# gmum/3d-point-clouds-autocomplete

Hardware: AMD Instinct MI355X
Metric: train-step point-clouds/sec at B=64, N=2048 (Chamfer+EMD) (higher is better)
Workload: dtype f32 storage / accumulation / results; matrix products formed from f16 x2 (bf16 x3) pieces of the fp32 operands — NOT IEEE-fp32 products: the all-fp32-kernel step is `value_strict_fp32`

## Files before the change

3d-point-clouds-autocomplete_amd/csrc/hp_skinny.h:

```cpp
#pragma once
#include <hip/hip_runtime.h>

#define HP_SK_MAX_OPS 16

enum { HP_SK_F = 1, HP_SK_X = 2, HP_SK_W = 3, HP_SK_FIN = 4 };

typedef struct HpSkSrc {
    const float* p;
    long slab;
    const float* bias;
    const float* mask;
    float* mat;
    int S, ld, ldm, ldmat, relu;
} HpSkSrc;

typedef struct HpSkOp {
    int type, phase;
    HpSkSrc a;
    const float* w;
    float* out;
    long out_slab;
    const float* out_bias;
    float* rsum;
    int w_ld, out_ld, out_relu;
    int M, N, K, CL;
    int ntasks;
} HpSkOp;

typedef struct HpSkProgram {
    int nops;
    HpSkOp op[HP_SK_MAX_OPS];
} HpSkProgram;

#ifdef __cplusplus
int hp_skinny_run(HpSkProgram* prog, hipStream_t stream);
int hp_skinny_check(HpSkProgram* prog);
bool hp_skinny_enabled();
#endif
```

3d-point-clouds-autocomplete_amd/csrc/model.hip:

```cpp
#include "hp_common.h"
#include "hp_gemm.h"
#include "hp_conv_split.h"
#include "hp_model.h"
#include "hp_skinny.h"
#include "hp_enc_bwd.h"
#include <algorithm>
#include <cstdlib>

extern "C" int hp_gemm_f32(const HpGemmDesc* d, hipStream_t stream);
extern "C" int hp_gemm_tile_rows(const HpGemmDesc* d);
extern "C" int hp_colsum_f32(int batch, int M, int N, const float* X, long sXz, int ldx, const float* mask, long sMaskz,
                             int ldmask, float* out, long sOz, float* ws, hipStream_t stream);

namespace {

constexpr int kEnc[6] = {3, 64, 128, 256, 512, 512};
constexpr int kTrunk[5] = {64, 128, 512, 1024, 2048};
constexpr long kSplitWs = 4L << 20;

#define TRY(x)            \
    do {                  \
        int _rc = (x);    \
        if (_rc) return _rc; \
    } while (0)
// ... 913 lines not shown
                                  const HpEncoderGrads* gr, float* ws, const float* fwd_ws, int dedup, hipStream_t stream) {
    const HpEncoderBwdIO io{x, w, eps, argidx, g, f, lv, grad_out, grad_mu, grad_explv, gr, ws, fwd_ws, is_vae, grad_out_ld};
    return encoder_backward_impl(B, Np, out_size, 1, &io, dedup, stream);
}
HP_API int hp_encoder_backward(int B, int Np, const float* x, const HpEncoderWeights* w, int out_size, int is_vae,
                               const float* eps, const int* argidx, const float* g, const float* f, const float* lv,
                               const float* grad_out, const float* grad_mu, const float* grad_explv,
                               const HpEncoderGrads* gr, float* ws, const float* fwd_ws, int dedup, hipStream_t stream) {
    return hp_encoder_backward_ld(B, Np, x, w, out_size, is_vae, eps, argidx, g, f, lv, grad_out, out_size, grad_mu, grad_explv, gr, ws,
                                  fwd_ws, dedup, stream);
}
HP_API int hp_encoder_backward_set_fused(int on) { return g_enc_bwd_fused.set(on); }
HP_API int hp_encoder_backward_set_chain_f16(int on) { return hp_enc_bwd_chain_f16_set(on); }
HP_API int hp_encoder_backward_pair(int B, int Np, int out_size, const HpEncoderBwdIO* io, int dedup, hipStream_t stream) {
    return encoder_backward_impl(B, Np, out_size, 2, io, dedup, stream);
}

HP_API int hp_encoder_plan(int B, int Np, int out_size, int n, const int* is_vae, const int* ld, int aligned, int dedup,
                           HpEncoderPlan* plan) {
    HP_CHECK_ARG(n >= 1 && n <= 2 && is_vae && plan && enc_fwd_shape_ok(B, Np, out_size, n));
    for (int z = 0; z < n; ++z) HP_CHECK_ARG(!ld || ld[z] == 0 || ld[z] >= out_size);
    HP_CHECK_ARG(!dedup || (long)Np * 512 < (1L << 31));
    *plan = HpEncoderPlan{};
    float* const base = reinterpret_cast<float*>(uintptr_t(1) << 40);
    const long span = 1L << 34;
    HpEncoderWeights w{};
    HpEncoderGrads gr{};
    for (int l = 0; l < 5; ++l) {
        w.conv_w[l] = w.conv_b[l] = base;
        gr.conv_w[l] = gr.conv_b[l] = base;
    }
    w.fc_w = w.fc_b = w.mu_w = w.mu_b = w.std_w = w.std_b = base;
    gr.fc_w = gr.fc_b = gr.mu_w = gr.mu_b = gr.std_w = gr.std_b = base;
    auto ld_of = [&](int z) { return (ld && ld[z] > 0) ? ld[z] : out_size; };

    const EncFwdRoute r = enc_fwd_route(B, Np, out_size, n);
    plan->conv_format = r.presplit ? HP_ENC_CONV_PFORMAT : r.split ? HP_ENC_CONV_SPLIT_F32 : HP_ENC_CONV_GEMM_F32;
    plan->pool_fused = r.fused ? 1 : 0;
    plan->tile_rows = r.tr;
    if (enc_fwd_tails_try_skinny(r, B)) {
        EncTail t[2];
        for (int z = 0; z < n; ++z) {
            const bool block = n > 1 && !is_vae[z];
            t[z] = EncTail{base, &w, is_vae[z], base, base + (block ? out_size : 0), base, base + (z + 1) * span + r.tail_off,
                           block ? ld_of(z) : out_size};
        }
        HpSkProgram pr;
        plan->fwd_tails_skinny = enc_tail_forward_program(B, out_size, n, t, pr) == 0 && hp_skinny_check(&pr) == 0;
    }

    plan->bwd_fused = (enc_bwd_shapes_fuse(B, out_size, dedup) && aligned) ? 1 : 0;
    const bool chain16 = hp_enc_bwd_chain_f16_enabled();
    plan->bwd_splits = plan->bwd_fused ? enc_bwd_splits(B, chain16) : 0;
    EncTailBwd t[2];
    bool ask = true;
    for (int z = 0; z < n; ++z) {
        const EncBwdWs L = enc_bwd_layout(base + (z + 1) * span + (aligned ? 0 : 1), B, out_size);
        const float* dmu_p = is_vae[z] ? L.dmu : base + (n > 1 ? out_size : 0);
        const int dmu_ld = is_vae[z] ? out_size : ld_of(z);
        t[z] = EncTailBwd{base, base, &w, dmu_p, dmu_ld, is_vae[z] ? L.dlv : nullptr, &gr, L.dfc, L.dg, L.split};
        ask = ask && enc_bwd_tail_try_skinny(B, dmu_p, dmu_ld);
        if (!plan->bwd_fused) {
            HpSkProgram pr;
            plan->bwd_tails_skinny[z] = enc_bwd_tail_try_skinny(B, dmu_p, dmu_ld) &&
                                        enc_tail_backward_program(B, out_size, 1, &t[z], pr) == 0 && hp_skinny_check(&pr) == 0;
        }
    }
    if (plan->bwd_fused) {
        HpSkProgram pr;
        const int ok = ask && enc_tail_backward_program(B, out_size, n, t, pr) == 0 && hp_skinny_check(&pr) == 0;
        for (int z = 0; z < n; ++z) plan->bwd_tails_skinny[z] = ok;
    }
    return 0;
}

namespace {
template <typename P>
bool heads_contiguous(P const* hw, P const* hb, const int* out, int n) {
    for (int h = 0; h + 1 < n; ++h)
        if (hw[h + 1] != hw[h] + (long)out[h] * 2048 || hb[h + 1] != hb[h] + out[h]) return false;
    return n > 0;
}

int trunk_forward_skinny(int B, int in_size, const float* latent, const HpHyperWeights* w, float* t, float* slabs,
                         hipStream_t stream) {
    if (B > 64 || in_size % 32) return -2;
    HpSkProgram pr{};
    HpSkSrc src{};
    src.p = latent; src.S = 1; src.ld = in_size;
    float* tl = t;
    float* sl = slabs;
    int kin = in_size;
    for (int l = 0; l < 5; ++l) {
        const int N = kTrunk[l];
        const int S = sk_ranges(kin, N / 32, 4);
        HpSkOp& op = pr.op[pr.nops++];
        op.type = HP_SK_F; op.phase = l;
        op.a = src;
        op.w = w->trunk_w[l]; op.w_ld = kin;
        op.M = B; op.N = N; op.K = kin; op.CL = kin / S;
        op.out_ld = N;
        HpSkSrc next{};
        next.ld = N;
        if (S == 1) {
            op.out = tl; op.out_bias = w->trunk_b[l]; op.out_relu = l < 4;
            next.p = tl; next.S = 1;
        } else {
            op.out = sl; op.out_slab = 64L * N;
            next.p = sl; next.slab = 64L * N; next.S = S; next.bias = w->trunk_b[l]; next.relu = l < 4;
            next.mat = tl; next.ldmat = N;
            sl += (long)S * 64 * N;
            if (sl - slabs > kSplitWs) return -2;
        }
        src = next;
        kin = N;
        tl += (long)B * N;
    }
    if (src.S > 1) {
        HpSkOp& op = pr.op[pr.nops++];
        op.type = HP_SK_FIN; op.phase = 5;
        op.out = src.mat; op.out_ld = src.ldmat;
        src.mat = nullptr;
        op.a = src;
        op.M = B; op.N = 2048; op.K = 1;
    }
    return hp_skinny_run(&pr, stream);
}

int trunk_backward_skinny(int B, int in_size, const float* latent, const HpHyperWeights* w, const float* const* act,
                          float* const* dt, const HpHyperGrads* gr, float* grad_latent, float* slabs, hipStream_t stream) {
    if (B > 64 || in_size % 32) return -2;
    HpSkProgram pr{};
    HpSkSrc src{};
    src.p = dt[4]; src.S = 1; src.ld = kTrunk[4];
    float* sl = slabs;
    int phase = 0;
    auto dw_op = [&](int l) {
        HpSkOp& op = pr.op[pr.nops++];
        op.type = HP_SK_W; op.phase = phase;
        op.a.p = dt[l]; op.a.S = 1; op.a.ld = kTrunk[l];
        op.w = l ? act[l - 1] : latent; op.w_ld = l ? kTrunk[l - 1] : in_size;
        op.out = gr->trunk_w[l]; op.out_ld = op.w_ld; op.rsum = gr->trunk_b[l];
        op.M = B; op.N = kTrunk[l]; op.K = op.w_ld;
    };
    for (int l = 4; l >= 0; --l, ++phase) {
        const int N = kTrunk[l], K = l ? kTrunk[l - 1] : in_size;
        if (l == 0 && !grad_latent) {
            HpSkOp& op = pr.op[pr.nops++];
            op.type = HP_SK_FIN; op.phase = phase;
            op.out = src.mat; op.out_ld = src.ldmat;
            src.mat = nullptr;
            op.a = src;
            op.M = B; op.N = N; op.K = 1;
        } else {
            const int S = sk_ranges(N, K / 32, 4);
            HpSkOp& op = pr.op[pr.nops++];
            op.type = HP_SK_X; op.phase = phase;
            op.a = src;
            op.w = w->trunk_w[l]; op.w_ld = K;
            op.M = B; op.N = N; op.K = K; op.CL = N / S;
            op.out_ld = K;
            HpSkSrc next{};
            next.ld = K;
            if (l == 0) {
                if (S == 1) {
                    op.out = grad_latent;
                } else {
                    op.out = sl; op.out_slab = 64L * K;
                    next.p = sl; next.slab = 64L * K; next.S = S;
                    sl += (long)S * 64 * K;
                }
            } else {
                op.out = sl; op.out_slab = 64L * K;
                next.p = sl; next.slab = 64L * K; next.S = S;
                next.mask = act[l - 1]; next.ldm = K; next.mat = dt[l - 1]; next.ldmat = K;
                sl += (long)S * 64 * K;
            }
            if (sl - slabs > kSplitWs) return -2;
            src = next;
        }
        if (l == 4) dw_op(4);
        else if (l <= 2) dw_op(l + 1);
    }
    if (grad_latent && src.p && src.S > 1) {
        HpSkOp& op = pr.op[pr.nops++];
        op.type = HP_SK_FIN; op.phase = phase;
        op.a = src;
        op.out = grad_latent; op.out_ld = in_size;
        op.M = B; op.N = in_size; op.K = 1;
    }
    dw_op(0);
    return hp_skinny_run(&pr, stream);
}

template <typename T>
inline T* hyper_splitws(T* t, int B) { return t + ((long)B * (64 + 128 + 512 + 1024 + 2048) + 3) / 4 * 4; }
inline int heads_total(const HpHyperWeights* w) {
    int total = 0;
    for (int hd = 0; hd < w->n_heads; ++hd) total += w->head_out[hd];
    return total;
}
int heads_fwd_route(int B, const HpHyperWeights* w, const float* t) {
    if (!heads_contiguous(w->head_w, w->head_b, w->head_out, w->n_heads)) return HP_HEADS_FWD_PER_HEAD;
    const float* t5 = t + (long)B * (64 + 128 + 512 + 1024);
    return hp_heads_fwd_enabled() && hp_heads_fwd_ws_floats() <= kSplitWs &&
                   hp_heads_fwd_ok(B, heads_total(w), 2048, t5, w->head_w[0], hyper_splitws(t, B))
               ? HP_HEADS_FWD_STREAM : HP_HEADS_FWD_GEMM;
}
int heads_dw_route(const HpHyperWeights* w, const HpHyperGrads* gr, const float* t5) {
    const bool skip_dw = gr->head_w[0] == nullptr;
    bool gb_contig = true;
    for (int h = 0; h + 1 < w->n_heads; ++h) gb_contig = gb_contig && gr->head_b[h + 1] == gr->head_b[h] + w->head_out[h];
    const bool w_contig = heads_contiguous(w->head_w, w->head_b, w->head_out, w->n_heads);
    if (skip_dw) return gb_contig && w_contig ? HP_HEADS_DW_SKIPPED : -1;
    if (!w_contig || !heads_contiguous(gr->head_w, gr->head_b, w->head_out, w->n_heads)) return HP_HEADS_DW_PER_HEAD;
    return hp_heads_dw_fast_ok(2048, t5, gr->head_w[0]) ? HP_HEADS_DW_DIRECT : HP_HEADS_DW_GEMM;
}
int heads_dw_rows_route(const float* t5_all, const float* dW_rows) {
    return hp_heads_dw_fast_ok(2048, t5_all, dW_rows) ? HP_HEADS_DW_DIRECT : HP_HEADS_DW_GEMM;
}
}

HP_API long hp_hypernet_saved_floats(int B) { return (long)B * (64 + 128 + 512 + 1024 + 2048) + kSplitWs + 64; }
HP_API long hp_hypernet_backward_workspace_floats(int B) { return (long)B * (64 + 128 + 512 + 1024 + 2048) + kSplitWs + 64; }

HP_API int hp_hypernet_set_heads_stream(int on) { return hp_heads_fwd_set(on); }

HP_API int hp_hypernet_forward(int B, int in_size, const float* latent, const HpHyperWeights* w, float* t, float* theta,
                               int theta_ld, hipStream_t stream) {
    HP_CHECK_ARG(B > 0 && in_size > 0 && latent && w && t && theta && w->n_heads > 0 && w->n_heads <= HP_MAX_HEADS);
    Op op{stream, hyper_splitws(t, B)};
    const float* in = latent;
    int kin = in_size;
    float* tl = t;
    int sk = hp_skinny_enabled() ? trunk_forward_skinny(B, in_size, latent, w, t, op.splitws, stream) : -2;
    if (sk != -2) {
        TRY(sk);
        in = t + (long)B * (64 + 128 + 512 + 1024);
    } else {
        for (int l = 0; l < 5; ++l) {
            TRY(op.lin_fwd(in, 0, kin, w->trunk_w[l], 0, w->trunk_b[l], 0, tl, 0, kTrunk[l], B, kTrunk[l], kin, 1, l < 4));
            in = tl;
            kin = kTrunk[l];
            tl += (long)B * kTrunk[l];
        }
    }
    const int total = heads_total(w);
    HP_CHECK_ARG(total <= theta_ld);
    switch (heads_fwd_route(B, w, t)) {
    case HP_HEADS_FWD_STREAM:
        TRY(hp_heads_fwd(B, total, in, w->head_w[0], w->head_b[0], theta, theta_ld, op.splitws, stream));
        break;
    case HP_HEADS_FWD_GEMM:
        TRY(op.lin_fwd(in, 0, 2048, w->head_w[0], 0, w->head_b[0], 0, theta, 0, theta_ld, B, total, 2048, 1, false));
        break;
    default: {
        int off = 0;
        for (int hd = 0; hd < w->n_heads; ++hd) {
            TRY(op.lin_fwd(in, 0, 2048, w->head_w[hd], 0, w->head_b[hd], 0, theta + off, 0, theta_ld, B, w->head_out[hd], 2048,
                           1, false));
            off += w->head_out[hd];
        }
    }
    }
    HP_RETURN_LAST_ERROR();
}

namespace {
int hypernet_backward_impl(int B, int in_size, const float* latent, const HpHyperWeights* w, const float* t, const float* grad_theta,
                           int theta_ld, const HpHyperGrads* gr, float* grad_latent, float* ws, hipStream_t stream, hipStream_t after);
}
HP_API int hp_hypernet_backward(int B, int in_size, const float* latent, const HpHyperWeights* w, const float* t,
                                const float* grad_theta, int theta_ld, const HpHyperGrads* gr, float* grad_latent, float* ws,
                                hipStream_t stream) {
    return hypernet_backward_impl(B, in_size, latent, w, t, grad_theta, theta_ld, gr, grad_latent, ws, stream, nullptr);
}
HP_API int hp_hypernet_backward_ordered(int B, int in_size, const float* latent, const HpHyperWeights* w, const float* t,
                                        const float* grad_theta, int theta_ld, const HpHyperGrads* gr, float* grad_latent, float* ws,
                                        hipStream_t stream, hipStream_t after) {
    return hypernet_backward_impl(B, in_size, latent, w, t, grad_theta, theta_ld, gr, grad_latent, ws, stream, after);
}
namespace {
int hypernet_backward_impl(int B, int in_size, const float* latent, const HpHyperWeights* w, const float* t, const float* grad_theta,
                           int theta_ld, const HpHyperGrads* gr, float* grad_latent, float* ws, hipStream_t stream, hipStream_t after) {
    HP_CHECK_ARG(B > 0 && in_size > 0 && latent && w && t && grad_theta && gr && ws);
    const float* act[5];
    {
        const float* tl = t;
        for (int l = 0; l < 5; ++l) {
            act[l] = tl;
            tl += (long)B * kTrunk[l];
        }
    }
    float* p = ws;
    float* dt[5];
    for (int l = 0; l < 5; ++l) {
        dt[l] = p;
        p += (long)B * kTrunk[l];
    }
    Op op{stream, p};
    int off = 0;
    const int total = heads_total(w);
    const int route = heads_dw_route(w, gr, act[4]);
    HP_CHECK_ARG(route >= 0);
    const bool fused = route != HP_HEADS_DW_PER_HEAD;
    if (fused) {
        if (route == HP_HEADS_DW_DIRECT) {
// ... 150 lines not shown
```

3d-point-clouds-autocomplete_amd/csrc/skinny.hip:

```cpp
#include "hp_common.h"
#include "hp_pieces.h"
#include "hp_skinny.h"
#include <algorithm>
#include <atomic>
#include <cstdlib>

namespace {

using namespace hp_pieces;
typedef int i32x4 __attribute__((ext_vector_type(4)));

constexpr int kThreads = 256;
constexpr int kCLMax = 128;
constexpr int kLdsFloats = 96 * (kCLMax + 4);

constexpr int kPhaseOps = 8;
struct Prog {
    int nops;
    HpSkOp op[kPhaseOps];
};

struct Buf {
    __amdgpu_buffer_rsrc_t r;
    __device__ __forceinline__ explicit Buf(const void* base)
        : r(__builtin_amdgcn_make_buffer_rsrc(const_cast<void*>(base), 0, 0x7fffffff, 0x00020000)) {}
    __device__ __forceinline__ float4 ld4(long off_floats) const {
        const i32x4 v = __builtin_amdgcn_raw_buffer_load_b128(r, (int)(off_floats * 4), 0, 0);
        return make_float4(__int_as_float(v.x), __int_as_float(v.y), __int_as_float(v.z), __int_as_float(v.w));
    }
    __device__ __forceinline__ float ld1(long off_floats) const {
        return __int_as_float(__builtin_amdgcn_raw_buffer_load_b32(r, (int)(off_floats * 4), 0, 0));
    }
};

__device__ __forceinline__ float4 f4add(float4 a, float4 b) { return make_float4(a.x + b.x, a.y + b.y, a.z + b.z, a.w + b.w); }
__device__ __forceinline__ float4 f4zero() { return make_float4(0.f, 0.f, 0.f, 0.f); }
__device__ __forceinline__ float f4get(const float4& v, int s) { return s == 0 ? v.x : (s == 1 ? v.y : (s == 2 ? v.z : v.w)); }

__device__ __forceinline__ float4 src_finish(const HpSkSrc& a, float4 v, const float4& aux) {
    if (a.bias) v = f4add(v, aux);
    if (a.relu) v = make_float4(fmaxf(v.x, 0.f), fmaxf(v.y, 0.f), fmaxf(v.z, 0.f), fmaxf(v.w, 0.f));
    if (a.mask) v = make_float4(aux.x > 0.f ? v.x : 0.f, aux.y > 0.f ? v.y : 0.f, aux.z > 0.f ? v.z : 0.f, aux.w > 0.f ? v.w : 0.f);
    return v;
}

__device__ __forceinline__ float4 src_load4(const HpSkSrc& a, int row, int c) {
    const Buf buf(a.p);
    const long off = (long)row * a.ld + c;
    float4 t[4];
#pragma unroll
    for (int s = 0; s < 4; ++s)
        if (s < a.S) t[s] = buf.ld4(off + (long)s * a.slab);
    float4 aux = f4zero();
    if (a.bias) aux = *reinterpret_cast<const float4*>(a.bias + c);
    if (a.mask) aux = *reinterpret_cast<const float4*>(a.mask + (long)row * a.ldm + c);
    float4 v = t[0];
#pragma unroll
    for (int s = 1; s < 4; ++s)
        if (s < a.S) v = f4add(v, t[s]);
    return src_finish(a, v, aux);
}

template <int NG, int SB>
struct SrcChunk {
    static constexpr int CL = NG * 16, ldl = CL + 4, QR = CL / 4;
    float4 t[NG][SB], aux[NG];
    int c0;
    __device__ __forceinline__ void load(const HpSkSrc& a, int M, int c0_) {
        c0 = c0_;
        const Buf buf(a.p);
        const float* auxp = a.bias ? a.bias : (a.mask ? a.mask : a.p);
        const int aux_ld = a.bias ? 0 : (a.mask ? a.ldm : a.ld);
#pragma unroll
        for (int e = 0; e < NG; ++e) {
            const int idx = threadIdx.x + e * kThreads, row = min(idx / QR, M - 1), q = idx % QR;
            const long off = (long)row * a.ld + c0 + 4 * q;
#pragma unroll
            for (int u = 0; u < SB; ++u) t[e][u] = buf.ld4(off + (long)(u < a.S ? u : 0) * a.slab);
            aux[e] = *reinterpret_cast<const float4*>(auxp + (long)row * aux_ld + c0 + 4 * q);
        }
    }
    __device__ __forceinline__ void store(const HpSkSrc& a, int M, float* As, bool materialise) const {
#pragma unroll
        for (int e = 0; e < NG; ++e) {
            const int idx = threadIdx.x + e * kThreads, row = idx / QR, q = idx % QR;
            float4 v = t[e][0];
#pragma unroll
            for (int u = 1; u < SB; ++u)
                if (u < a.S) v = f4add(v, t[e][u]);
            float4 f = src_finish(a, v, aux[e]);
            if (row >= M) f = f4zero();
            *reinterpret_cast<float4*>(&As[row * ldl + 4 * q]) = f;
            if (materialise && row < M) *reinterpret_cast<float4*>(a.mat + (long)row * a.ldmat + c0 + 4 * q) = f;
        }
    }
};

template <int NG>
struct WChunk {
    static constexpr int CL = NG * 16, ldl = CL + 4, QR = CL / 4, NV = NG / 2;
    static_assert(NV * kThreads == 32 * QR, "whole passes of the workgroup over the block");
    float4 v[NV];
    __device__ __forceinline__ void load(const float* __restrict__ W, int ld, int N, int n0, int c0) {
#pragma unroll
        for (int e = 0; e < NV; ++e) {
            const int idx = threadIdx.x + e * kThreads;
            v[e] = *reinterpret_cast<const float4*>(W + (long)min(n0 + idx / QR, N - 1) * ld + c0 + 4 * (idx % QR));
        }
    }
    __device__ __forceinline__ void store(float* Ws) const {
#pragma unroll
        for (int e = 0; e < NV; ++e) {
            const int idx = threadIdx.x + e * kThreads;
            *reinterpret_cast<float4*>(&Ws[(idx / QR) * ldl + 4 * (idx % QR)]) = v[e];
        }
    }
};

__device__ __forceinline__ void reduce_store(f32x16 (&acc)[2], float* red, const HpSkOp& op, float* out, int ncols, int col0,
                                             bool direct) {
    const int lane = threadIdx.x & 63, w = threadIdx.x >> 6, i = lane & 31, h = lane >> 5;
    __syncthreads();
#pragma unroll
    for (int mt = 0; mt < 2; ++mt)
#pragma unroll
        for (int e = 0; e < 16; ++e) red[((w * 2 + mt) * 16 + e) * 64 + lane] = acc[mt][e];
    __syncthreads();
    const int col = col0 + i;
    const float bv = (direct && op.out_bias && col < ncols) ? op.out_bias[col] : 0.f;
#pragma unroll
    for (int mt = 0; mt < 2; ++mt)
#pragma unroll
        for (int q = 0; q < 4; ++q) {
            const int e = 4 * w + q;
            float v = red[((0 * 2 + mt) * 16 + e) * 64 + lane];
            v += red[((1 * 2 + mt) * 16 + e) * 64 + lane];
            v += red[((2 * 2 + mt) * 16 + e) * 64 + lane];
            v += red[((3 * 2 + mt) * 16 + e) * 64 + lane];
            const int row = mt * 32 + cd_row(e, h);
            if (direct) {
                v += bv;
                if (op.out_relu) v = fmaxf(v, 0.f);
            }
            if (row < op.M && col < ncols) out[(long)row * op.out_ld + col] = v;
        }
    __syncthreads();
}

template <int NG, int SB>
__device__ __forceinline__ void task_f(const HpSkOp& op, int t, float* lds) {
    constexpr int CL = NG * 16, ldl = CL + 4, ks = CL / 4;
    const int strips = (op.N + 31) >> 5;
    const int strip = t % strips, range = t / strips;
    const int nr = op.K / op.CL;
    const int lane = threadIdx.x & 63, w = threadIdx.x >> 6, i = lane & 31, h = lane >> 5;
    const int chunks = op.CL / CL;
    const bool mat = strip == 0 && op.a.mat != nullptr;
    float* As = lds;
    float* Ws = lds + 64 * ldl;
    f32x16 acc[2] = {};
    SrcChunk<NG, SB> sc[2];
    WChunk<NG> wc[2];
    const int c_first = range * op.CL;
    auto mfma_chunk = [&]() {
#pragma unroll
        for (int kq = 0; kq < ks / 8; ++kq) {
            const int kk = w * ks + kq * 8;
            const float4 a0 = *reinterpret_cast<const float4*>(&As[i * ldl + kk + 4 * h]);
            const float4 a1 = *reinterpret_cast<const float4*>(&As[(32 + i) * ldl + kk + 4 * h]);
            const float4 bb = *reinterpret_cast<const float4*>(&Ws[i * ldl + kk + 4 * h]);
#pragma unroll
            for (int s = 0; s < 4; ++s) {
                acc[0] = __builtin_amdgcn_mfma_f32_32x32x2f32(f4get(a0, s), f4get(bb, s), acc[0], 0, 0, 0);
                acc[1] = __builtin_amdgcn_mfma_f32_32x32x2f32(f4get(a1, s), f4get(bb, s), acc[1], 0, 0, 0);
            }
        }
    };
    wc[0].load(op.w, op.w_ld, op.N, strip * 32, c_first);
    sc[0].load(op.a, op.M, c_first);
#pragma unroll 1
    for (int ch = 0; ch < chunks; ch += 2) {
        {
            const int c1 = c_first + min(ch + 1, chunks - 1) * CL;
            wc[1].load(op.w, op.w_ld, op.N, strip * 32, c1);
            sc[1].load(op.a, op.M, c1);
        }
        if (ch) __syncthreads();
        sc[0].store(op.a, op.M, As, mat);
        wc[0].store(Ws);
        __syncthreads();
        mfma_chunk();
        if (ch + 1 >= chunks) break;
        {
            const int c2 = c_first + min(ch + 2, chunks - 1) * CL;
            wc[0].load(op.w, op.w_ld, op.N, strip * 32, c2);
            sc[0].load(op.a, op.M, c2);
        }
// ... 36 lines not shown
#pragma unroll
            for (int s = 0; s < 4; ++s) {
                acc[0] = __builtin_amdgcn_mfma_f32_32x32x2f32(f4get(a0, s), bwc[4 * g + s], acc[0], 0, 0, 0);
                acc[1] = __builtin_amdgcn_mfma_f32_32x32x2f32(f4get(a1, s), bwc[4 * g + s], acc[1], 0, 0, 0);
            }
        }
    };
    const int n_first = range * op.CL;
    load_b(n_first, bw[0]);
    sc[0].load(op.a, op.M, n_first);
#pragma unroll 1
    for (int ch = 0; ch < chunks; ch += 2) {
        {
            const int n1 = n_first + min(ch + 1, chunks - 1) * CL;
            load_b(n1, bw[1]);
            sc[1].load(op.a, op.M, n1);
        }
        if (ch) __syncthreads();
        sc[0].store(op.a, op.M, As, mat);
        __syncthreads();
        mfma_chunk(bw[0]);
        if (ch + 1 >= chunks) break;
        {
            const int n2 = n_first + min(ch + 2, chunks - 1) * CL;
            load_b(n2, bw[0]);
            sc[0].load(op.a, op.M, n2);
        }
        __syncthreads();
        sc[1].store(op.a, op.M, As, mat);
        __syncthreads();
        mfma_chunk(bw[1]);
    }
    reduce_store(acc, lds, op, op.out + (long)range * op.out_slab, op.K, unit * 32, nr == 1);
}

__device__ __forceinline__ void task_w(const HpSkOp& op, int t) {
    const int lane = threadIdx.x & 63, w = threadIdx.x >> 6, i = lane & 31, h = lane >> 5;
    const int ktiles = (op.K + 31) >> 5, ntiles = (op.N + 31) >> 5;
    const int tile = t * 4 + w;
    if (tile >= ktiles * ntiles) return;
    const int kt = tile % ktiles, nt = tile / ktiles;
    const int ncol = min(nt * 32 + i, op.N - 1), kcol = min(kt * 32 + i, op.K - 1);
    const float* ap = op.a.p + ncol;
    const float* bp = op.w + kcol;
    float av[32], bv[32];
#pragma unroll
    for (int s = 0; s < 32; ++s) {
        const int m = min(2 * s + h, op.M - 1);
        av[s] = ap[(long)m * op.a.ld];
        bv[s] = bp[(long)m * op.w_ld];
    }
#pragma unroll
    for (int s = 0; s < 32; ++s)
        if (2 * s + h >= op.M) av[s] = 0.f;
    f32x16 acc = {};
    float asum = 0.f;
#pragma unroll
    for (int s = 0; s < 32; ++s) {
        asum += av[s];
        acc = __builtin_amdgcn_mfma_f32_32x32x2f32(av[s], bv[s], acc, 0, 0, 0);
    }
    if (op.rsum && kt == 0) {
        const float other = __shfl_xor(asum, 32, 64);
        if (h == 0 && nt * 32 + i < op.N) op.rsum[nt * 32 + i] = asum + other;
    }
    const int col = kt * 32 + i;
    if (col < op.K) {
#pragma unroll
        for (int e = 0; e < 16; ++e) {
            const int row = nt * 32 + cd_row(e, h);
            if (row < op.N) op.out[(long)row * op.out_ld + col] = acc[e];
        }
    }
}

__device__ __forceinline__ void task_fin(const HpSkOp& op, int t) {
    const int q_per_row = op.N >> 2;
    const int idx = t * kThreads + threadIdx.x;
    if (idx >= op.M * q_per_row) return;
    const int r = idx / q_per_row, q = idx - r * q_per_row;
    *reinterpret_cast<float4*>(op.out + (long)r * op.out_ld + 4 * q) = src_load4(op.a, r, 4 * q);
}

template <bool LIGHT>
__global__ __launch_bounds__(kThreads) void skinny_kernel(const Prog g_arg) {
    __shared__ __attribute__((aligned(16))) float lds[LIGHT ? 4 : kLdsFloats];
    const int G = gridDim.x;
    const Prog& g = *(const Prog*)__builtin_amdgcn_kernarg_segment_ptr();
    (void)g_arg;
    int base = 0;
    for (int o = 0; o < g.nops; ++o) {
        const HpSkOp& op = g.op[o];
        int first = (int)blockIdx.x - base % G;
        if (first < 0) first += G;
        const int cl = min(op.CL, kCLMax);
        for (int t = first; t < op.ntasks; t += G) {
            if (!LIGHT && op.type == HP_SK_F) {
                if (op.a.S == 1) {
                    if (cl == 128) task_f<8, 1>(op, t, lds);
                    else if (cl == 64) task_f<4, 1>(op, t, lds);
                    else task_f<2, 1>(op, t, lds);
                } else {
                    if (cl >= 64) task_f<4, 4>(op, t, lds);
                    else task_f<2, 4>(op, t, lds);
                }
            } else if (!LIGHT && op.type == HP_SK_X) {
                if (op.a.S == 1) {
                    if (cl == 128) task_x<8, 1>(op, t, lds);
                    else if (cl == 64) task_x<4, 1>(op, t, lds);
                    else task_x<2, 1>(op, t, lds);
                } else {
                    if (cl >= 64) task_x<4, 4>(op, t, lds);
                    else task_x<2, 4>(op, t, lds);
                }
            } else if (op.type == HP_SK_W) {
                task_w(op, t);
            } else if (op.type == HP_SK_FIN) {
                task_fin(op, t);
            }
        }
        base += op.ntasks;
    }
}

inline bool aligned16(const void* q) { return (reinterpret_cast<uintptr_t>(q) & 15) == 0; }
inline bool pow2(int v) { return v > 0 && (v & (v - 1)) == 0; }

bool src_ok(const HpSkSrc& a, int cols) {
    if (!a.p || a.S < 1 || a.S > 4 || !aligned16(a.p) || a.ld % 4 || cols % 4) return false;
    if (a.S > 1 && a.slab % 4) return false;
    if (a.bias && !aligned16(a.bias)) return false;
    if (a.mask && (!aligned16(a.mask) || a.ldm % 4)) return false;
    if (a.mat && (!aligned16(a.mat) || a.ldmat % 4)) return false;
    if (a.bias && a.mask) return false;
    return true;
}

}

namespace {
hp::Switch g_skinny("HP_SKINNY", 1);
}
bool hp_skinny_enabled() { return g_skinny.get() != 0; }
HP_API int hp_skinny_set_enabled(int on) { return g_skinny.set(on); }

namespace {
std::atomic<long> g_programs_run{0};
}
HP_API long hp_skinny_programs_run(void) { return g_programs_run.load(std::memory_order_relaxed); }

int hp_skinny_check(HpSkProgram* prog) {
    if (!prog || prog->nops < 1 || prog->nops > HP_SK_MAX_OPS) return -2;
    int maxtasks = 0, phases = 1;
    for (int o = 0; o < prog->nops; ++o) {
        HpSkOp& op = prog->op[o];
        if (o && op.phase < prog->op[o - 1].phase) return -2;
        if (o && op.phase != prog->op[o - 1].phase) ++phases;
        if (op.M < 1 || op.M > 64 || op.N < 1 || op.K < 1 || !op.out || !aligned16(op.out)) return -2;
        switch (op.type) {
            case HP_SK_F:
                if (op.K % 32 || !pow2(op.CL) || op.CL < 32 || op.K % op.CL || !src_ok(op.a, op.K) || !op.w || !aligned16(op.w) ||
                    op.w_ld % 4)
                    return -2;
                op.ntasks = ((op.N + 31) / 32) * (op.K / op.CL);
                break;
            case HP_SK_X:
                if (op.N % 32 || !pow2(op.CL) || op.CL < 32 || op.N % op.CL || !src_ok(op.a, op.N) || !op.w) return -2;
                op.ntasks = ((op.K + 31) / 32) * (op.N / op.CL);
                break;
            case HP_SK_W:
                if (!op.a.p || op.a.S != 1 || op.a.bias || op.a.mask || op.a.relu || !op.w) return -2;
                op.ntasks = (((op.N + 31) / 32) * ((op.K + 31) / 32) + 3) / 4;
                break;
            case HP_SK_FIN:
                if (op.N % 4 || op.out_ld % 4 || !src_ok(op.a, op.N)) return -2;
                op.ntasks = (op.M * (op.N / 4) + kThreads - 1) / kThreads;
                break;
            default: return -2;
        }
        maxtasks = std::max(maxtasks, op.ntasks);
    }
    (void)phases;
    (void)maxtasks;
    return 0;
}

int hp_skinny_run(HpSkProgram* prog, hipStream_t stream) {
    if (hp_skinny_check(prog)) return -2;
    g_programs_run.fetch_add(1, std::memory_order_relaxed);
    for (int b = 0; b < prog->nops;) {
        Prog g;
        g.nops = 0;
        int e = b, tasks = 0;
        bool light = true;
        for (; e < prog->nops && prog->op[e].phase == prog->op[b].phase && g.nops < kPhaseOps; ++e) {
            g.op[g.nops++] = prog->op[e];
            tasks += prog->op[e].ntasks;
            light = light && (prog->op[e].type == HP_SK_W || prog->op[e].type == HP_SK_FIN);
        }
        const dim3 grid(std::max(1, std::min(tasks, 512)));
        if (light) hipLaunchKernelGGL(skinny_kernel<true>, grid, dim3(kThreads), 0, stream, g);
        else hipLaunchKernelGGL(skinny_kernel<false>, grid, dim3(kThreads), 0, stream, g);
        b = e;
    }
    HP_RETURN_LAST_ERROR();
}
```

include/hyperpocket_hip.h:

```cpp
#ifndef HYPERPOCKET_HIP_H
#define HYPERPOCKET_HIP_H

#ifdef __cplusplus
extern "C" {
#endif

typedef struct ihipStream_t* hpStream_t;


int hp_nndistance(int b, int n, const float* xyz, int m, const float* xyz2, float* result, int* result_i,
                  float* result2, int* result2_i, hpStream_t stream);

int hp_nn_set_queries_per_lane(int r);
int hp_nn_queries_per_lane(int b, int n, int m);

int hp_nndistancegrad(int b, int n, const float* xyz1, int m, const float* xyz2, const float* grad_dist1,
                      const int* idx1, const float* grad_dist2, const int* idx2, float* grad_xyz1, float* grad_xyz2,
                      hpStream_t stream);

int hp_approxmatch(int b, int n, int m, const float* xyz1, const float* xyz2, float* match, float* temp,
                   hpStream_t stream);
long hp_approxmatch_workspace_floats(int b, int n, int m);
int hp_approxmatch_ws(int b, int n, int m, const float* xyz1, const float* xyz2, float* match, float* temp, float* ws,
                      hpStream_t stream);
// ... 142 lines not shown
int hp_conv_presplit_set(int on);
long hp_gemm_pp_workspace_floats(long M, int N, int K);
int hp_gemm_pp_prepare(long M, int N, int K, int xcb, const float* X, const float* W, float* ws, hpStream_t stream);
int hp_gemm_pp_run(long M, int N, int K, int xcb, const float* bias, int relu, int mode, int group_rows, float* ws, hpStream_t stream);
int hp_gemm_pp_unpack(long M, int N, int K, const float* ws, float* C, hpStream_t stream);
int hp_gemm_pp_partials(long M, int N, int K, const float* ws, float* cmax, int* cidx, hpStream_t stream);
int hp_gemm_pp_plan(long M, int N, int mode, int n, int out[6]);
long hp_encoder_backward_workspace_floats(int B, int out_size);
int hp_encoder_backward(int B, int Np, const float* x, const HpEncoderWeights* w, int out_size, int is_vae,
                        const float* eps, const int* argidx, const float* g, const float* f, const float* lv,
                        const float* grad_out, const float* grad_mu, const float* grad_explv, const HpEncoderGrads* grads,
                        float* ws, const float* fwd_ws, int dedup, hpStream_t stream);
int hp_encoder_backward_ld(int B, int Np, const float* x, const HpEncoderWeights* w, int out_size, int is_vae,
                           const float* eps, const int* argidx, const float* g, const float* f, const float* lv,
                           const float* grad_out, int grad_out_ld, const float* grad_mu, const float* grad_explv,
                           const HpEncoderGrads* grads, float* ws, const float* fwd_ws, int dedup, hpStream_t stream);
typedef struct HpEncoderBwdIO {
    const float* x;
    const HpEncoderWeights* w;
    const float* eps;
    const int* argidx;
    const float *g, *f, *lv;
    const float *grad_out, *grad_mu, *grad_explv;
    const HpEncoderGrads* gr;
    float* ws;
    const float* fwd_ws;
    int is_vae;
    int grad_out_ld;
} HpEncoderBwdIO;
int hp_encoder_backward_pair(int B, int Np, int out_size, const HpEncoderBwdIO* io , int dedup, hpStream_t stream);
enum { HP_ENC_CONV_PFORMAT = 0, HP_ENC_CONV_SPLIT_F32 = 1, HP_ENC_CONV_GEMM_F32 = 2 };
typedef struct HpEncoderPlan {
    int conv_format;
    int pool_fused;
    int tile_rows;
    int fwd_tails_skinny;
    int bwd_fused;
    int bwd_splits;
    int bwd_tails_skinny[2];
} HpEncoderPlan;
int hp_encoder_plan(int B, int Np, int out_size, int n, const int* is_vae, const int* ld, int aligned, int dedup,
                    HpEncoderPlan* plan);
int hp_encoder_backward_set_fused(int on);
int hp_encoder_backward_set_chain_f16(int on);
int hp_conv_split_set(int on);
long hp_gemm_f16x2_workspace_floats(long M, int N, int K);
int hp_gemm_f16x2_prepare(long M, int N, int K, const float* X, const float* W, float* ws, hpStream_t stream);
int hp_gemm_f16x2_run(long M, int N, int K, const float* X, const float* bias, float* C, int relu, const float* ws, hpStream_t stream);

int hp_hypernet_set_heads_stream(int on);
long hp_hypernet_saved_floats(int B);
int hp_hypernet_forward(int B, int in_size, const float* latent, const HpHyperWeights* w, float* t, float* theta,
                        int theta_ld, hpStream_t stream);
long hp_hypernet_backward_workspace_floats(int B);
int hp_hypernet_backward(int B, int in_size, const float* latent, const HpHyperWeights* w, const float* t,
                         const float* grad_theta, int theta_ld, const HpHyperGrads* grads, float* grad_latent ,
                         float* ws, hpStream_t stream);
int hp_hypernet_backward_ordered(int B, int in_size, const float* latent, const HpHyperWeights* w, const float* t,
                                 const float* grad_theta, int theta_ld, const HpHyperGrads* grads, float* grad_latent ,
                                 float* ws, hpStream_t stream, hpStream_t after);
long hp_hypernet_t5_offset(int B);
long hp_hypernet_heads_dw_workspace_floats(void);
int hp_hypernet_heads_dw_rows(int Kc, int rows, int r0, const float* dtheta_all, int theta_ld, const float* t5_all,
                              float* dW_rows, float* ws, hpStream_t stream);
enum { HP_HEADS_FWD_STREAM = 0, HP_HEADS_FWD_GEMM = 1, HP_HEADS_FWD_PER_HEAD = 2 };
enum { HP_HEADS_DW_DIRECT = 0, HP_HEADS_DW_GEMM = 1, HP_HEADS_DW_PER_HEAD = 2, HP_HEADS_DW_SKIPPED = 3 };
typedef struct HpHeadsPlan {
    int fwd_route;
    int dw_route;
    int dw_rows_route;
} HpHeadsPlan;
int hp_hypernet_heads_plan(int B, const HpHyperWeights* w, const HpHyperGrads* grads , const float* t,
                           const float* dW_rows , HpHeadsPlan* plan);

int hp_hypernet_heads_dw_adam(int Kc, int rows, int r0, const float* dtheta_all, int theta_ld, const float* t5_all,
                              float* W_rows, float* m_rows, float* v_rows, float lr, float beta1, float beta2, float eps,
                              int step, hpStream_t stream);
int hp_hypernet_heads_dw_adam_bg(int Kc, int rows, int r0, const float* dtheta_all, int theta_ld, const float* t5_all,
                                 float* W_rows, float* m_rows, float* v_rows, float lr, float beta1, float beta2, float eps,
                                 int step, int cus, hpStream_t stream);

int hp_skinny_set_enabled(int on);
long hp_skinny_programs_run(void);

long hp_target_theta_size(int n_hidden, const int* channels);
long hp_target_saved_floats(int B, int N, int n_hidden, const int* channels);
int hp_target_forward(int B, int N, int n_hidden, const int* channels, const float* theta, int theta_ld, const float* pts,
                      float* acts, float* y, hpStream_t stream);
long hp_target_backward_workspace_floats(int B, int N, int n_hidden, const int* channels);
int hp_target_backward(int B, int N, int n_hidden, const int* channels, const float* theta, int theta_ld, const float* pts,
                       const float* acts, const float* grad_y, float* grad_theta, float* ws, hpStream_t stream);

int hp_target_fused_supported(int n_hidden, const int* channels);
long hp_target_fused_workspace_floats(int B, int N);
int hp_target_fused_set_f16(int on);
int hp_target_fused_forward(int B, int N, const float* theta, int theta_ld, const float* pts, float* y, hpStream_t stream);
int hp_target_fused_backward(int B, int N, const float* theta, int theta_ld, const float* pts, const float* grad_y,
                             float* grad_theta, float* ws, hpStream_t stream);

int hp_sample_points(long total, float coef, unsigned long long seed, unsigned long long offset, float* out,
                     hpStream_t stream);
int hp_slice_clouds(int B, int N, int target, const float* pts, unsigned long long seed, int max_rounds, float* part_a,
                    float* part_b, float* plane, int* status, hpStream_t stream);
int hp_slice_clouds_planes(int B, int N, int target, const float* pts, const double* planes, int R, float* part_a,
                           float* part_b, int* plane_idx, int* status, hpStream_t stream);
long hp_make_batch_workspace_bytes(int B, int N);
int hp_make_batch(int M, int N, int target, const float* clouds, int B, const int* ids, const long long* streams,
                  const int* degrees, const float* rot, unsigned long long seed, int max_candidates, int groups,
                  float* existing, float* missing, float* gt, float* plane, int* index, int* failed, void* ws,
                  hpStream_t stream);
#define HP_VIEW_SPLIT_MAX_POINTS 8192
#define HP_VIEW_SPLIT_MIN_RESOLUTION 4
#define HP_VIEW_SPLIT_MAX_RESOLUTION 128
#define HP_VIEW_SPLIT_MAX_WINDOW 4
int hp_make_view_batch_plan(int N, int R, int* threads, int* lds);
int hp_make_view_batch(int M, int N, int target, const float* clouds, int B, const int* ids, const float* frames ,
                       const int* degrees, const float* rot, double dist, double scale, int R, int w, float* existing,
                       float* missing, float* gt, unsigned char* side , float* occlusion ,
                       hpStream_t stream);
#define HP_SCAN_MAX_POINTS (1 << 22)
int hp_scan_boxes(int S, const float* points, const long long* offsets, float* center , float* scale ,
                  hpStream_t stream);
int hp_prepare_scans(int B, const float* points, const long long* offsets, int S, const int* ids, const long long* streams,
                     unsigned long long seed, int target, int replace, const float* center, const float* scale, float* out,
                     int* index, int* failed, hpStream_t stream);
int hp_restore_scans(int K, int N, const float* completions, const float* s_scale, const float* center, const float* scale,
                     float* out, hpStream_t stream);
#define HP_FPS_MAX_POINTS 8192
int hp_farthest_points(int B, int P, const float* clouds, const int* counts, const int* start, int k, int* index,
                       float* radius2, int* failed, hpStream_t stream);
int hp_farthest_points_plan(int P, int* threads, int* points_per_lane);
#define HP_KNN_MAX_POINTS 65536
int hp_knn_points(int S, const float* points, const long long* offsets, const float* queries, const long long* query_offsets,
                  int k, int exclude_self, int* index , float* dist2 , hpStream_t stream);
int hp_knn_points_plan(int k, int* instance_k, int* threads, int* tile);
int hp_scan_outliers(int S, const float* points, const long long* offsets, int k, float ratio, unsigned char* keep ,
                     float* mean_dist , int* kept , hpStream_t stream);
#define HP_KNN_GRID_MAX_POINTS (1 << 22)
long long hp_knn_grid_workspace_bytes(int S, long long T, long long Q);
int hp_knn_grid_plan(int k, int* instance_k, int* threads, int* tile);
int hp_knn_grid(int S, const float* points, const long long* offsets, const float* queries, const long long* query_offsets,
                int k, int exclude_self, const float* cell , int* index , float* dist2 ,
                float* mean_dist , float* grid , void* ws, long long ws_bytes,
                hpStream_t stream);
int hp_outlier_keep(int S, const float* mean_dist, const long long* offsets, float ratio, unsigned char* keep ,
                    int* kept , hpStream_t stream);
int hp_scan_outliers_grid(int S, const float* points, const long long* offsets, int k, float ratio, const float* cell,
                          unsigned char* keep , float* mean_dist , int* kept , void* ws,
                          long long ws_bytes, hpStream_t stream);
#define HP_CLUSTER_MAX_POINTS 32768
int hp_scan_clusters(int S, const float* points, const long long* offsets, float radius, int max_points,
                     int* label , int* size , int* clusters , int* largest ,
                     hpStream_t stream);
int hp_scan_clusters_plan(int max_points, int* threads, int* tile, int* lds_bytes);
#define HP_PLANE_MAX_TRIALS 4096
long hp_scan_plane_workspace_bytes(int S, int trials);
int hp_scan_plane_plan(int trials, int* threads, int* rows_per_lane, int* trial_tile);
int hp_scan_plane(int S, const float* points, const long long* offsets, const long long* streams ,
                  unsigned long long seed, int trials, float threshold, int min_inliers, float min_share,
                  int* trial , int* inliers , int* found , int* sample ,
                  float* sample_plane , unsigned char* inlier , long long* moments ,
                  int* shift , void* ws, hpStream_t stream);
int hp_scan_plane_side(int S, const float* points, const long long* offsets, const float* planes , float threshold,
                       float* dist , unsigned char* keep , int* kept , hpStream_t stream);
#define HP_VOXEL_GRID_HALF (1 << 20)
long hp_scan_voxels_workspace_bytes(long long T, int slots_per_row);
// ... 112 lines not shown
```

Baseline: 28790.

## Specialize skinny kernel instances per phase body set to cut LDS and raise occupancy

Replaces the two-way light/heavy skinny kernel with six template instances. Each instance compiles only the task bodies its launch phase actually uses, and sizes its LDS allocation and launch-bounds occupancy hint to match. Phases that use only small-CL bodies can then keep two workgroups per CU with a smaller LDS footprint instead of the worst-case 96x132 buffer. It also adds a planning API for inspecting which instance each launch picks. The costs are more compiled kernel variants and the risk that the tighter launch bounds raise register pressure or cause spills for the larger bodies.

```diff
diff --git a/3d-point-clouds-autocomplete_amd/csrc/hp_skinny.h b/3d-point-clouds-autocomplete_amd/csrc/hp_skinny.h
--- a/3d-point-clouds-autocomplete_amd/csrc/hp_skinny.h
+++ b/3d-point-clouds-autocomplete_amd/csrc/hp_skinny.h
@@ -32,7 +32,21 @@
     HpSkOp op[HP_SK_MAX_OPS];
 } HpSkProgram;
 
+enum {
+    HP_SK_BODY_F81 = 1 << 0, HP_SK_BODY_F41 = 1 << 1, HP_SK_BODY_F21 = 1 << 2, HP_SK_BODY_F44 = 1 << 3, HP_SK_BODY_F24 = 1 << 4,
+    HP_SK_BODY_X81 = 1 << 5, HP_SK_BODY_X41 = 1 << 6, HP_SK_BODY_X21 = 1 << 7, HP_SK_BODY_X44 = 1 << 8, HP_SK_BODY_X24 = 1 << 9
+};
+#define HP_SK_INSTANCES 6
+
+typedef struct HpSkPlan {
+    int launches;
+    int instance[HP_SK_MAX_OPS];
+    unsigned bodies[HP_SK_MAX_OPS];
+    int workgroups[HP_SK_MAX_OPS];
+} HpSkPlan;
+
 #ifdef __cplusplus
+int hp_skinny_plan(HpSkProgram* prog, HpSkPlan* plan);
 int hp_skinny_run(HpSkProgram* prog, hipStream_t stream);
 int hp_skinny_check(HpSkProgram* prog);
 bool hp_skinny_enabled();
diff --git a/3d-point-clouds-autocomplete_amd/csrc/model.hip b/3d-point-clouds-autocomplete_amd/csrc/model.hip
--- a/3d-point-clouds-autocomplete_amd/csrc/model.hip
+++ b/3d-point-clouds-autocomplete_amd/csrc/model.hip
@@ -1019,10 +1019,10 @@
     return n > 0;
 }
 
-int trunk_forward_skinny(int B, int in_size, const float* latent, const HpHyperWeights* w, float* t, float* slabs,
-                         hipStream_t stream) {
+int trunk_forward_program(int B, int in_size, const float* latent, const HpHyperWeights* w, float* t, float* slabs,
+                          HpSkProgram& pr) {
     if (B > 64 || in_size % 32) return -2;
-    HpSkProgram pr{};
+    pr = HpSkProgram{};
     HpSkSrc src{};
     src.p = latent; src.S = 1; src.ld = in_size;
     float* tl = t;
@@ -1061,13 +1061,19 @@
         op.a = src;
         op.M = B; op.N = 2048; op.K = 1;
     }
+    return 0;
+}
+int trunk_forward_skinny(int B, int in_size, const float* latent, const HpHyperWeights* w, float* t, float* slabs,
+                         hipStream_t stream) {
+    HpSkProgram pr;
+    if (trunk_forward_program(B, in_size, latent, w, t, slabs, pr)) return -2;
     return hp_skinny_run(&pr, stream);
 }
 
-int trunk_backward_skinny(int B, int in_size, const float* latent, const HpHyperWeights* w, const float* const* act,
-                          float* const* dt, const HpHyperGrads* gr, float* grad_latent, float* slabs, hipStream_t stream) {
+int trunk_backward_program(int B, int in_size, const float* latent, const HpHyperWeights* w, const float* const* act,
+                           float* const* dt, const HpHyperGrads* gr, float* grad_latent, float* slabs, HpSkProgram& pr) {
     if (B > 64 || in_size % 32) return -2;
-    HpSkProgram pr{};
+    pr = HpSkProgram{};
     HpSkSrc src{};
     src.p = dt[4]; src.S = 1; src.ld = kTrunk[4];
     float* sl = slabs;
@@ -1127,6 +1133,12 @@
         op.M = B; op.N = in_size; op.K = 1;
     }
     dw_op(0);
+    return 0;
+}
+int trunk_backward_skinny(int B, int in_size, const float* latent, const HpHyperWeights* w, const float* const* act,
+                          float* const* dt, const HpHyperGrads* gr, float* grad_latent, float* slabs, hipStream_t stream) {
+    HpSkProgram pr;
+    if (trunk_backward_program(B, in_size, latent, w, act, dt, gr, grad_latent, slabs, pr)) return -2;
     return hp_skinny_run(&pr, stream);
 }
 
@@ -1160,6 +1172,40 @@
 
 HP_API long hp_hypernet_saved_floats(int B) { return (long)B * (64 + 128 + 512 + 1024 + 2048) + kSplitWs + 64; }
 HP_API long hp_hypernet_backward_workspace_floats(int B) { return (long)B * (64 + 128 + 512 + 1024 + 2048) + kSplitWs + 64; }
+
+HP_API int hp_skinny_program_plan(int kind, int B, int size, int n, const int* is_vae, int want_latent, HpSkPlan* plan) {
+    HP_CHECK_ARG(kind >= 0 && kind <= 3 && B > 0 && size > 0 && plan);
+    HP_CHECK_ARG(kind < 2 || (n >= 1 && n <= 2 && is_vae));
+    float* const base = reinterpret_cast<float*>(uintptr_t(1) << 40);
+    HpSkProgram pr;
+    if (kind < 2) {
+        HpHyperWeights w{};
+        HpHyperGrads gr{};
+        const float* act[5];
+        float* dt[5];
+        for (int l = 0; l < 5; ++l) {
+            w.trunk_w[l] = w.trunk_b[l] = base;
+            gr.trunk_w[l] = gr.trunk_b[l] = base;
+            act[l] = dt[l] = base;
+        }
+        const int rc = kind == 0 ? trunk_forward_program(B, size, base, &w, base, base, pr)
+                                 : trunk_backward_program(B, size, base, &w, act, dt, &gr, want_latent ? base : nullptr, base, pr);
+        if (rc) return -2;
+    } else {
+        HpEncoderWeights w{};
+        HpEncoderGrads gr{};
+        w.fc_w = w.fc_b = w.mu_w = w.mu_b = w.std_w = w.std_b = base;
+        gr.fc_w = gr.fc_b = gr.mu_w = gr.mu_b = gr.std_w = gr.std_b = base;
+        EncTail tf[2];
+        EncTailBwd tb[2];
+        for (int z = 0; z < n; ++z) {
+            tf[z] = EncTail{base, &w, is_vae[z], base, base, base, base, size};
+            tb[z] = EncTailBwd{base, base, &w, base, size, is_vae[z] ? base : nullptr, &gr, base, base, base};
+        }
+        if (kind == 2 ? enc_tail_forward_program(B, size, n, tf, pr) : enc_tail_backward_program(B, size, n, tb, pr)) return -2;
+    }
+    return hp_skinny_plan(&pr, plan);
+}
 
 HP_API int hp_hypernet_set_heads_stream(int on) { return hp_heads_fwd_set(on); }
 
diff --git a/3d-point-clouds-autocomplete_amd/csrc/skinny.hip b/3d-point-clouds-autocomplete_amd/csrc/skinny.hip
--- a/3d-point-clouds-autocomplete_amd/csrc/skinny.hip
+++ b/3d-point-clouds-autocomplete_amd/csrc/skinny.hip
@@ -12,7 +12,29 @@
 
 constexpr int kThreads = 256;
 constexpr int kCLMax = 128;
-constexpr int kLdsFloats = 96 * (kCLMax + 4);
+constexpr int kRedFloats = 4 * 2 * 16 * 64;
+
+constexpr unsigned kF81 = HP_SK_BODY_F81, kF41 = HP_SK_BODY_F41, kF21 = HP_SK_BODY_F21, kF44 = HP_SK_BODY_F44, kF24 = HP_SK_BODY_F24;
+constexpr unsigned kX81 = HP_SK_BODY_X81, kX41 = HP_SK_BODY_X41, kX21 = HP_SK_BODY_X21, kX44 = HP_SK_BODY_X44, kX24 = HP_SK_BODY_X24;
+constexpr unsigned kFSmall = kF41 | kF21 | kF24, kFAll = kFSmall | kF81 | kF44;
+constexpr unsigned kXSmall = kX41 | kX21 | kX24, kXAll = kXSmall | kX81 | kX44;
+constexpr unsigned kAllBodies = kFAll | kXAll;
+constexpr unsigned kInstanceSet[HP_SK_INSTANCES] = {0u, kFSmall, kXSmall, kFAll, kXAll, kAllBodies};
+
+__host__ __device__ inline unsigned op_body(int type, int CL, int S) {
+    const int cl = CL < kCLMax ? CL : kCLMax;
+    if (type == HP_SK_F) return S == 1 ? (cl == 128 ? kF81 : cl == 64 ? kF41 : kF21) : (cl >= 64 ? kF44 : kF24);
+    if (type == HP_SK_X) return S == 1 ? (cl == 128 ? kX81 : cl == 64 ? kX41 : kX21) : (cl >= 64 ? kX44 : kX24);
+    return 0u;
+}
+constexpr int set_wg_per_cu(unsigned set) { return !set ? 4 : (set & (kF81 | kF44 | kX81 | kX44)) ? 1 : 2; }
+constexpr int set_lds_floats(unsigned set) {
+    if (!set) return 4;
+    const int cl = (set & (kF81 | kX81)) ? 128 : 64;
+    const int rows = (set & kFAll) ? 96 : 64;
+    return rows * (cl + 4) > kRedFloats ? rows * (cl + 4) : kRedFloats;
+}
+static_assert(2 * set_lds_floats(kFSmall) * 4 <= 160 * 1024 && set_lds_floats(kAllBodies) * 4 <= 64 * 1024, "LDS per CU / per workgroup");
 
 constexpr int kPhaseOps = 8;
 struct Prog {
@@ -100,19 +122,19 @@
 struct WChunk {
     static constexpr int CL = NG * 16, ldl = CL + 4, QR = CL / 4, NV = NG / 2;
     static_assert(NV * kThreads == 32 * QR, "whole passes of the workgroup over the block");
-    float4 v[NV];
+    f32x4 v[NV];
     __device__ __forceinline__ void load(const float* __restrict__ W, int ld, int N, int n0, int c0) {
 #pragma unroll
         for (int e = 0; e < NV; ++e) {
             const int idx = threadIdx.x + e * kThreads;
-            v[e] = *reinterpret_cast<const float4*>(W + (long)min(n0 + idx / QR, N - 1) * ld + c0 + 4 * (idx % QR));
+            v[e] = *reinterpret_cast<const f32x4*>(W + (long)min(n0 + idx / QR, N - 1) * ld + c0 + 4 * (idx % QR));
         }
     }
     __device__ __forceinline__ void store(float* Ws) const {
 #pragma unroll
         for (int e = 0; e < NV; ++e) {
             const int idx = threadIdx.x + e * kThreads;
-            *reinterpret_cast<float4*>(&Ws[(idx / QR) * ldl + 4 * (idx % QR)]) = v[e];
+            *reinterpret_cast<f32x4*>(&Ws[(idx / QR) * ldl + 4 * (idx % QR)]) = v[e];
         }
     }
 };
@@ -315,9 +337,10 @@
     *reinterpret_cast<float4*>(op.out + (long)r * op.out_ld + 4 * q) = src_load4(op.a, r, 4 * q);
 }
 
-template <bool LIGHT>
-__global__ __launch_bounds__(kThreads) void skinny_kernel(const Prog g_arg) {
-    __shared__ __attribute__((aligned(16))) float lds[LIGHT ? 4 : kLdsFloats];
+template <unsigned SET>
+__global__ __launch_bounds__(kThreads, set_wg_per_cu(SET)) void skinny_kernel(const Prog g_arg) {
+    constexpr bool LIGHT = SET == 0;
+    __shared__ __attribute__((aligned(16))) float lds[set_lds_floats(SET)];
     const int G = gridDim.x;
     const Prog& g = *(const Prog*)__builtin_amdgcn_kernarg_segment_ptr();
     (void)g_arg;
@@ -326,31 +349,20 @@
         const HpSkOp& op = g.op[o];
         int first = (int)blockIdx.x - base % G;
         if (first < 0) first += G;
-        const int cl = min(op.CL, kCLMax);
+        const unsigned body = LIGHT ? 0u : op_body(op.type, op.CL, op.a.S);
         for (int t = first; t < op.ntasks; t += G) {
-            if (!LIGHT && op.type == HP_SK_F) {
-                if (op.a.S == 1) {
-                    if (cl == 128) task_f<8, 1>(op, t, lds);
-                    else if (cl == 64) task_f<4, 1>(op, t, lds);
-                    else task_f<2, 1>(op, t, lds);
-                } else {
-                    if (cl >= 64) task_f<4, 4>(op, t, lds);
-                    else task_f<2, 4>(op, t, lds);
-                }
-            } else if (!LIGHT && op.type == HP_SK_X) {
-                if (op.a.S == 1) {
-                    if (cl == 128) task_x<8, 1>(op, t, lds);
-                    else if (cl == 64) task_x<4, 1>(op, t, lds);
-                    else task_x<2, 1>(op, t, lds);
-                } else {
-                    if (cl >= 64) task_x<4, 4>(op, t, lds);
-                    else task_x<2, 4>(op, t, lds);
-                }
-            } else if (op.type == HP_SK_W) {
-                task_w(op, t);
-            } else if (op.type == HP_SK_FIN) {
-                task_fin(op, t);
-            }
+            if ((SET & kF81) && body == kF81) task_f<8, 1>(op, t, lds);
+            else if ((SET & kF41) && body == kF41) task_f<4, 1>(op, t, lds);
+            else if ((SET & kF21) && body == kF21) task_f<2, 1>(op, t, lds);
+            else if ((SET & kF44) && body == kF44) task_f<4, 4>(op, t, lds);
+            else if ((SET & kF24) && body == kF24) task_f<2, 4>(op, t, lds);
+            else if ((SET & kX81) && body == kX81) task_x<8, 1>(op, t, lds);
+            else if ((SET & kX41) && body == kX41) task_x<4, 1>(op, t, lds);
+            else if ((SET & kX21) && body == kX21) task_x<2, 1>(op, t, lds);
+            else if ((SET & kX44) && body == kX44) task_x<4, 4>(op, t, lds);
+            else if ((SET & kX24) && body == kX24) task_x<2, 4>(op, t, lds);
+            else if (op.type == HP_SK_W) task_w(op, t);
+            else if (op.type == HP_SK_FIN) task_fin(op, t);
         }
         base += op.ntasks;
     }
@@ -418,23 +430,81 @@
     return 0;
 }
 
+namespace {
+hp::Switch g_instances("HP_SKINNY_INSTANCES", 1);
+
+struct Launch {
+    int end, tasks, instance;
+    unsigned bodies;
+};
+Launch next_launch(const HpSkProgram* prog, int b, bool per_phase) {
+    Launch l{b, 0, HP_SK_INSTANCES - 1, 0u};
+    for (; l.end < prog->nops && prog->op[l.end].phase == prog->op[b].phase && l.end - b < kPhaseOps; ++l.end) {
+        const HpSkOp& op = prog->op[l.end];
+        l.tasks += op.ntasks;
+        l.bodies |= op_body(op.type, op.CL, op.a.S);
+    }
+    if (!l.bodies) l.instance = 0;
+    else if (per_phase)
+        for (int i = 0; i < HP_SK_INSTANCES; ++i)
+            if ((l.bodies & ~kInstanceSet[i]) == 0u) {
+                l.instance = i;
+                break;
+            }
+    return l;
+}
+
+template <unsigned SET>
+void launch(const Prog& g, dim3 grid, hipStream_t stream) {
+    hipLaunchKernelGGL(skinny_kernel<SET>, grid, dim3(kThreads), 0, stream, g);
+}
+}
+
+HP_API int hp_skinny_set_instances(int mode) { return g_instances.set(mode); }
+
+HP_API int hp_skinny_instance_info(int instance, unsigned* bodies, int* wg_per_cu, int* lds_bytes) {
+    HP_CHECK_ARG(instance >= 0 && instance < HP_SK_INSTANCES);
+    if (bodies) *bodies = kInstanceSet[instance];
+    if (wg_per_cu) *wg_per_cu = set_wg_per_cu(kInstanceSet[instance]);
+    if (lds_bytes) *lds_bytes = kInstanceSet[instance] ? set_lds_floats(kInstanceSet[instance]) * 4 : 0;
+    return 0;
+}
+
+int hp_skinny_plan(HpSkProgram* prog, HpSkPlan* plan) {
+    if (!plan || hp_skinny_check(prog)) return -2;
+    *plan = HpSkPlan{};
+    const bool per_phase = g_instances.get() != 0;
+    for (int b = 0; b < prog->nops;) {
+        const Launch l = next_launch(prog, b, per_phase);
+        plan->instance[plan->launches] = l.instance;
+        plan->bodies[plan->launches] = l.bodies;
+        plan->workgroups[plan->launches] = std::max(1, std::min(l.tasks, 512));
+        ++plan->launches;
+        b = l.end;
+    }
+    return 0;
+}
+
 int hp_skinny_run(HpSkProgram* prog, hipStream_t stream) {
     if (hp_skinny_check(prog)) return -2;
     g_programs_run.fetch_add(1, std::memory_order_relaxed);
+    const bool per_phase = g_instances.get() != 0;
     for (int b = 0; b < prog->nops;) {
+        const Launch l = next_launch(prog, b, per_phase);
         Prog g;
-        g.nops = 0;
-        int e = b, tasks = 0;
-        bool light = true;
-        for (; e < prog->nops && prog->op[e].phase == prog->op[b].phase && g.nops < kPhaseOps; ++e) {
-            g.op[g.nops++] = prog->op[e];
-            tasks += prog->op[e].ntasks;
-            light = light && (prog->op[e].type == HP_SK_W || prog->op[e].type == HP_SK_FIN);
-        }
-        const dim3 grid(std::max(1, std::min(tasks, 512)));
-        if (light) hipLaunchKernelGGL(skinny_kernel<true>, grid, dim3(kThreads), 0, stream, g);
-        else hipLaunchKernelGGL(skinny_kernel<false>, grid, dim3(kThreads), 0, stream, g);
-        b = e;
+        g.nops = l.end - b;
+        for (int o = b; o < l.end; ++o) g.op[o - b] = prog->op[o];
+        const dim3 grid(std::max(1, std::min(l.tasks, 512)));
+        switch (l.instance) {
+            case 0: launch<kInstanceSet[0]>(g, grid, stream); break;
+            case 1: launch<kInstanceSet[1]>(g, grid, stream); break;
+            case 2: launch<kInstanceSet[2]>(g, grid, stream); break;
+            case 3: launch<kInstanceSet[3]>(g, grid, stream); break;
+            case 4: launch<kInstanceSet[4]>(g, grid, stream); break;
+            default: launch<kInstanceSet[5]>(g, grid, stream); break;
+        }
+        b = l.end;
     }
     HP_RETURN_LAST_ERROR();
 }
+static_assert(HP_SK_INSTANCES == 6, "one case per instance above");
diff --git a/include/hyperpocket_hip.h b/include/hyperpocket_hip.h
--- a/include/hyperpocket_hip.h
+++ b/include/hyperpocket_hip.h
@@ -248,6 +248,20 @@
 
 int hp_skinny_set_enabled(int on);
 long hp_skinny_programs_run(void);
+int hp_skinny_set_instances(int mode);
+enum {
+    HP_SK_BODY_F81 = 1 << 0, HP_SK_BODY_F41 = 1 << 1, HP_SK_BODY_F21 = 1 << 2, HP_SK_BODY_F44 = 1 << 3, HP_SK_BODY_F24 = 1 << 4,
+    HP_SK_BODY_X81 = 1 << 5, HP_SK_BODY_X41 = 1 << 6, HP_SK_BODY_X21 = 1 << 7, HP_SK_BODY_X44 = 1 << 8, HP_SK_BODY_X24 = 1 << 9
+};
+#define HP_SK_INSTANCES 6
+int hp_skinny_instance_info(int instance, unsigned* bodies, int* wg_per_cu, int* lds_bytes);
+typedef struct HpSkinnyPlan {
+    int launches;
+    int instance[16];
+    unsigned bodies[16];
+    int workgroups[16];
+} HpSkinnyPlan;
+int hp_skinny_program_plan(int kind, int B, int size, int n, const int* is_vae, int want_latent, HpSkinnyPlan* plan);
 
 long hp_target_theta_size(int n_hidden, const int* channels);
 long hp_target_saved_floats(int B, int N, int n_hidden, const int* channels);
```

Result: no change. 28940 (median of 6 runs) (+0.5%).
